# JiakangC/Neural-Network-Based-PDE-Solver

Measured on NVIDIA B200. Metric: collocation points/sec per train step (fwd+Δu+param-grad), higher is better.
Workload: dtype f32

## Files before the change

neural-network-based-pde-solver_b200/csrc/pde_tc.cu:

```cuda
#include <cuda_runtime.h>
#include <stdint.h>
#include <stdio.h>
#include <stdlib.h>
#include <string.h>
#include <atomic>
#include <type_traits>

#include "pde_launch.h"
#include "pde_tc.h"
#include "pde_tc_core.cuh"

namespace pde {
namespace tc {

constexpr int TP = 64;
constexpr int HP = 64;
constexpr int NEPI = 8;
constexpr int NE = 4;
constexpr int NTHREADS = (NEPI + 4) * 32;
constexpr int MAXC = 6;
constexpr int COL_R0 = 0;
constexpr int COL_G = 384;
constexpr int COL_SMALL = 448;

struct TcArgs {
  int n_h, act, H;
  const float* params;
  const unsigned char* wimg;
  const float* X;
  long long n;
  int num_tiles;
  int prog, n_q, want_grad;
  EnvDev<float> env;
  float alpha, beta_const, energy_const, inv_n;
  const float* f;
  const float* beta;
  const float* energy;
  const float* seed;
// ... 221 lines not shown
    }
  }
  if constexpr (ORDER == 2) {
    n0b += LB * lapb;
    nj[1 + ND] = B * lapb;
  }
  nj[0] = n0b;
}

template <int D, int C>
struct SmemMap {
  static constexpr int LIMIT = 232448;
  static constexpr int set_bytes = 2 * C * TILE_BYTES;
  static constexpr int par_floats = D * 64 + 4 * 64 + 64 + 4;
  static constexpr int red_floats = (2 * 64 * C > 256) ? 2 * 64 * C : 256;
  static constexpr int rest = 4096 + 1024 * (D > 0 ? D : 1) + par_floats * 4 + 64 * D * 4 + 64 * C * 4 + red_floats * 4 + 128;
  static constexpr int shadow_if = 2 * C * 2048;
  static constexpr bool fits3 = 2 * set_bytes + 3 * 2 * TILE_BYTES + shadow_if + rest <= LIMIT;
  static constexpr bool fits2 = 2 * set_bytes + 2 * 2 * TILE_BYTES + shadow_if + rest <= LIMIT;
  static constexpr bool shadow = (C <= 5) && (fits3 || fits2);
  static constexpr int w_slots = (C <= 5) ? ((shadow && !fits3) ? 2 : 3) : 1;
  static constexpr int off_T1 = 0;
  static constexpr int off_T2 = off_T1 + set_bytes;
  static constexpr int off_W = off_T2 + set_bytes;
  static constexpr int w_bytes = w_slots * 2 * TILE_BYTES;
  static constexpr int off_Z0 = off_W + w_bytes;
  static constexpr int off_XT = off_Z0 + (shadow ? shadow_if : 0);
  static constexpr int off_E = off_XT + 4096;
  static constexpr int off_par = off_E + 1024 * (D > 0 ? D : 1);
  static constexpr int off_X = off_par + par_floats * 4;
  static constexpr int off_nb = off_X + 64 * D * 4;
  static constexpr int off_red = off_nb + 64 * C * 4;
  static constexpr int off_bar = off_red + red_floats * 4;
  static constexpr int total = off_bar + 128;
  static_assert(total <= LIMIT, "shared-memory plan does not fit");
};

__device__ __forceinline__ void sts32(uint32_t addr, uint32_t v) { asm volatile("st.shared.b32 [%0], %1;" ::"r"(addr), "r"(v) : "memory"); }
__device__ __forceinline__ void stsm_x4(uint32_t addr, uint32_t r0, uint32_t r1, uint32_t r2, uint32_t r3) {
  asm volatile("stmatrix.sync.aligned.m8n8.x4.shared.b16 [%0], {%1,%2,%3,%4};" ::"r"(addr), "r"(r0), "r"(r1), "r"(r2), "r"(r3) : "memory");
}
__device__ __forceinline__ uint64_t l2_policy_evict_last() {
  uint64_t p;
  asm volatile("createpolicy.fractional.L2::evict_last.b64 %0, 1.0;" : "=l"(p));
  return p;
}
__device__ __forceinline__ uint64_t l2_policy_evict_first() {
  uint64_t p;
  asm volatile("createpolicy.fractional.L2::evict_first.b64 %0, 1.0;" : "=l"(p));
  return p;
}
__device__ __forceinline__ void stash_store(float4* p, float4 v, uint64_t pol) {
  asm volatile("st.global.cg.L2::cache_hint.v4.f32 [%0], {%1,%2,%3,%4}, %5;" ::"l"(p), "f"(v.x), "f"(v.y), "f"(v.z), "f"(v.w), "l"(pol) : "memory");
// ... 89 lines not shown
  uint64_t* bar_chunk = reinterpret_cast<uint64_t*>(sm + SM::off_bar);
  uint64_t* bar_d = bar_chunk + 4;
  uint64_t* bar_w = bar_chunk + 5;
  uint64_t* bar_own = bar_chunk + 6;
  uint64_t* bar_wt = bar_chunk + 7;
  uint32_t* tmem_slot = reinterpret_cast<uint32_t*>(bar_chunk + 8);
  int* sTileEnd = reinterpret_cast<int*>(bar_chunk + 14);
  float* sMx = reinterpret_cast<float*>(bar_chunk + 10);

  const int tid = threadIdx.x, warp = tid >> 5, lane = tid & 31;
  const int n_h = a.n_h;
  constexpr int act = ACT;
  const bool do_bwd = a.want_grad != 0;
  const uint32_t sbase = smem_u32(sm);
  const uint32_t sT1 = sbase + SM::off_T1, sT2 = sbase + SM::off_T2, sWT = sbase + SM::off_W;
  const uint32_t sXT = sbase + SM::off_XT, sET = sbase + SM::off_E, sZ0 = sbase + SM::off_Z0;

  auto w_addr = [&](int l) { return sWT + (WS == 3 ? l - 1 : (WS == 2 ? (l == 2 ? 0 : 1) : 0)) * 2 * TILE_BYTES; };
  for (int i = tid; i < D * 64 + n_h * 64; i += NTHREADS) sPar[i] = a.params[i];
  for (int i = tid; i < 64 + 1; i += NTHREADS) sWL[i] = a.params[D * 64 + n_h * 64 + i];
  if (tid == 0 && a.mode == 0) {
    sWL[65] = a.energy ? a.energy[0] : a.energy_const;
    sWL[66] = (a.seed ? a.seed[0] : 1.f) * a.inv_n;
    sWL[67] = (a.seed && a.prog == PDE_PROG_RAYLEIGH ? a.seed[1] : 1.f) * a.inv_n;
  }
  for (int i = tid; i < (1024 * (D > 0 ? D : 1)) / 4; i += NTHREADS) {
    const int n = i / 256, w = i % 256;
    reinterpret_cast<uint32_t*>(sm + SM::off_E)[i] = ((w >> 5) == n) ? ONE_X2 : 0u;
  }
  for (int i = tid; i < 1024; i += NTHREADS) {
    const int t = (i / 256) & 1, w = i % 256;
    reinterpret_cast<uint32_t*>(sm + SM::off_XT)[i] = (t == 0 && (w >> 5) == D) ? ONE_X2 : 0u;
  }
  {
    const uint4* src = reinterpret_cast<const uint4*>(a.wimg);
    uint4* dst = reinterpret_cast<uint4*>(sm + SM::off_W);
    for (int l = 1; l <= (n_h - 1 < WS ? n_h - 1 : WS); ++l) {
      dst = reinterpret_cast<uint4*>(sm + SM::off_W + (w_addr(l) - sWT));
      for (int i = tid; i < 2 * TILE_BYTES / 16; i += NTHREADS) dst[i] = src[(l - 1) * (2 * TILE_BYTES / 16) + i];
    }
  }
  if (tid == 0) {
    for (int j = 0; j < 4; ++j) mbar_init(&bar_chunk[j], NEPI);
    mbar_init(bar_d, 1);
    mbar_init(bar_w, 1);
    mbar_init(bar_own, 1);
    mbar_init(bar_wt, 1);
// ... 28 lines not shown
    }
  };
#else
  auto TS = [](int) {};
  auto TSW = [](int) {};
#endif
  auto d_addr = [&](int r, int c) { return taddr_of(tmem, 16 * (c & 1), COL_R0 + 192 * r + 64 * (c >> 1)); };

  if (warp >= NEPI) {
    asm volatile("setmaxnreg.dec.sync.aligned.u32 88;");
    if (warp == NEPI) {
      constexpr uint32_t ID_FWD = make_idesc(64, 64, 0, 0);
      constexpr uint32_t ID_FWD2 = make_idesc(128, 64, 0, 0), ID_DG2 = make_idesc(128, 64, 0, 1);
      constexpr uint32_t ID_DG = make_idesc(64, 64, 0, 1);
      constexpr uint32_t ID_WG = make_idesc(64, 64, 1, 1);
      constexpr uint32_t ID_SM = make_idesc(64, 8, 1, 0);
      constexpr uint32_t TD = TILE_BYTES >> 4;
      const uint32_t tm = __shfl_sync(0xffffffffu, tmem, 0);
      const uint32_t kT1K = (sT1 >> 4) | DESC_K_LBO, kT1M = (sT1 >> 4) | DESC_MN_LBO;
      const uint32_t kT2K = (sT2 >> 4) | DESC_K_LBO, kT2M = (sT2 >> 4) | DESC_MN_LBO;
      const uint32_t kXT0 = (sXT >> 4) | DESC_K_LBO, kETK = (sET >> 4) | DESC_K_LBO;
      uint32_t ph_chunk = 0, ph_own = 0, ph_wt = 0;
      int reg = 0;
      int cur_w = 1;
      const uint32_t kZ0 = (sZ0 >> 4) | ((128u >> 4) << 16);
      constexpr uint32_t DESC_HI_Z0 = (256u >> 4) | (1u << 14);
      bool w_loading = false;
      auto start_w_load = [&](int l) {
        if (elect_one()) {
          asm volatile("mbarrier.arrive.expect_tx.shared::cta.b64 _, [%0], %1;" ::"r"(smem_u32(bar_wt)), "r"(2 * TILE_BYTES) : "memory");
          asm volatile("cp.async.bulk.shared::cluster.global.mbarrier::complete_tx::bytes [%0], [%1], %2, [%3];" ::"r"(w_addr(l)),
                       "l"(a.wimg + (size_t)(l - 1) * 2 * TILE_BYTES), "r"(2 * TILE_BYTES), "r"(smem_u32(bar_wt))
                       : "memory");
        }
        __syncwarp();
        cur_w = l;
// ... 3 lines not shown
        if (WRES) return;
        if (WS == 2 && l == 2) return;
        if (cur_w != l) {
          if (elect_one()) mma_commit(bar_own);
          __syncwarp();
          mbar_wait(bar_own, ph_own);
          ph_own ^= 1;
          start_w_load(l);
        }
        if (w_loading) {
          mbar_wait(bar_wt, ph_wt);
          ph_wt ^= 1;
          w_loading = false;
        }
      };
      for (int tile = tile_begin; tile < tile_end; ++tile) {
        for (int l = 1; l < n_h; ++l) {
          uint32_t kT1K_ = kT1K, kT1M_ = kT1M, kT2K_ = kT2K, kT2M_ = kT2M, kXT0_ = kXT0, kETK_ = kETK, kZ0_ = kZ0;
          if constexpr (C <= 4) asm volatile("" : "+r"(kT1K_), "+r"(kT1M_), "+r"(kT2K_), "+r"(kT2M_), "+r"(kXT0_), "+r"(kETK_), "+r"(kZ0_));
          const uint32_t kW = (w_addr(l) >> 4) | DESC_K_LBO;
          const uint32_t dbase = tm + COL_R0 + 192 * reg;
          need_w(l);
#pragma unroll
          for (int j = 0; j < 4; ++j) {
            mbar_wait(&bar_chunk[j], ph_chunk);
            tc_fence_after();
            TS(100 + 10 * l + j);
            if (WS == 2 && j == 0 && l == 2 && n_h - 1 == 3) start_w_load(3);
            if (elect_one()) {
#pragma unroll
              for (int c = 0; c < C; ++c) {
                if (ch_paired(c, C) && (c & 1)) continue;
                const uint32_t d = dbase + 64 * (c >> 1);
                const uint32_t ah = kT1K_ + (ch_base(c, C) >> 4) + 2 * j, al = ah + (ch_lo(c, C) >> 4);
                const uint32_t id = ch_paired(c, C) ? ID_FWD2 : ID_FWD;
                mma_k(d, ah, DESC_HI, kW + 2 * j, DESC_HI, id, j > 0 ? 1u : 0u);
                mma_k(d, al, DESC_HI, kW + 2 * j, DESC_HI, id, 1u);
                mma_k(d, ah, DESC_HI, kW + TD + 2 * j, DESC_HI, id, 1u);
              }
            }
            __syncwarp();
          }
          if (elect_one()) mma_commit(bar_d);
          __syncwarp();
          ph_chunk ^= 1;
          reg ^= 1;
        }
        if (!do_bwd) continue;
        for (int l = n_h - 1; l >= 1; --l) {
          uint32_t kT1K_ = kT1K, kT1M_ = kT1M, kT2K_ = kT2K, kT2M_ = kT2M, kXT0_ = kXT0, kETK_ = kETK, kZ0_ = kZ0;
          if constexpr (C <= 4) asm volatile("" : "+r"(kT1K_), "+r"(kT1M_), "+r"(kT2K_), "+r"(kT2M_), "+r"(kXT0_), "+r"(kETK_), "+r"(kZ0_));
          const uint32_t kW = (w_addr(l) >> 4) | DESC_MN_LBO;
          const uint32_t dbase = tm + COL_R0 + 192 * reg;
          need_w(l);
#pragma unroll
          for (int j = 0; j < 4; ++j) {
            mbar_wait(&bar_chunk[j], ph_chunk);
            tc_fence_after();
            TS(200 + 10 * l + j);
            if (WS == 2 && j == 0 && l == 2 && n_h - 1 == 3) start_w_load(1);
            if (SHADOW && j == 0 && l < n_h - 1) {
              if (elect_one()) {
#pragma unroll
                for (int c = 0; c < C; ++c) {
                  if (ch_paired(c, C) && (c & 1)) continue;
                  const uint32_t d = dbase + 64 * (c >> 1);
// ... 34 lines not shown
#pragma unroll
              for (int ks = 0; ks < 4; ++ks) {
                const uint32_t zh = kT2M_ + ((ch_base(c, C) + ks * ch_kstep_mn(c, C)) >> 4), zl = zh + (ch_lo(c, C) >> 4);
                const uint32_t ah = kT1M_ + ((ch_base(c, C) + ks * ch_kstep_mn(c, C)) >> 4), al = ah + (ch_lo(c, C) >> 4);
                mma_k(d, zl, ch_hi_mn(c, C), ah, ch_hi_mn(c, C), ID_WG, (c == 0 && ks == 0) ? 0u : 1u);
                mma_k(d, zh, ch_hi_mn(c, C), al, ch_hi_mn(c, C), ID_WG, 1u);
              }
            }
#pragma unroll
            for (int c = 0; c < C; ++c) {
#pragma unroll
              for (int ks = 0; ks < 4; ++ks)
                mma_k(d, kT2M_ + ((ch_base(c, C) + ks * ch_kstep_mn(c, C)) >> 4), ch_hi_mn(c, C),
                      kT1M_ + ((ch_base(c, C) + ks * ch_kstep_mn(c, C)) >> 4), ch_hi_mn(c, C), ID_WG, 1u);
            }
            const uint32_t db = tm + (16u << 16) + COL_SMALL + 8 * l;
#pragma unroll
            for (int ks = 0; ks < 4; ++ks)
              mma_k(db, kT2M_ + ((ch_lo(0, C) + ks * ch_kstep_mn(0, C)) >> 4), ch_hi_mn(0, C), kETK_ + 2 * ks, DESC_HI, ID_SM, ks == 0 ? 0u : 1u);
#pragma unroll
            for (int ks = 0; ks < 4; ++ks) mma_k(db, kT2M_ + ((ks * ch_kstep_mn(0, C)) >> 4), ch_hi_mn(0, C), kETK_ + 2 * ks, DESC_HI, ID_SM, 1u);
            mma_commit(bar_w);
          }
          __syncwarp();
          if (refill_next) {
            mbar_wait(bar_own, ph_own);
            ph_own ^= 1;
            start_w_load(l - 1);
          }
        }
        {
          uint32_t kT1K_ = kT1K, kT1M_ = kT1M, kT2K_ = kT2K, kT2M_ = kT2M, kXT0_ = kXT0, kETK_ = kETK, kZ0_ = kZ0;
          if constexpr (C <= 4) asm volatile("" : "+r"(kT1K_), "+r"(kT1M_), "+r"(kT2K_), "+r"(kT2M_), "+r"(kXT0_), "+r"(kETK_), "+r"(kZ0_));
#pragma unroll
          for (int j = 0; j < 4; ++j) mbar_wait(&bar_chunk[j], ph_chunk);
          tc_fence_after();
          ph_chunk ^= 1;
          if (elect_one()) {
            const uint32_t d = tm + (16u << 16) + COL_SMALL;
            const uint32_t kXTK = kXT0_ + ((tile & 1) << 7);
#pragma unroll
            for (int ks = 0; ks < 4; ++ks) {
              mma_k(d, kT2M_ + ((ch_lo(0, C) + ks * ch_kstep_mn(0, C)) >> 4), ch_hi_mn(0, C), kXTK + 2 * ks, DESC_HI, ID_SM, ks == 0 ? 0u : 1u);
              mma_k(d, kT2M_ + ((ks * ch_kstep_mn(0, C)) >> 4), ch_hi_mn(0, C), kXTK + 64 + 2 * ks, DESC_HI, ID_SM, 1u);
            }
#pragma unroll
            for (int i = 0; i < ND; ++i) {
#pragma unroll
              for (int ks = 0; ks < 4; ++ks)
                mma_k(d, kT2M_ + ((ch_base(1 + i, C) + ch_lo(1 + i, C) + ks * ch_kstep_mn(1 + i, C)) >> 4), ch_hi_mn(1 + i, C),
                      kETK_ + 64 * (dir0 + i) + 2 * ks, DESC_HI, ID_SM, 1u);
            }
#pragma unroll
            for (int ks = 0; ks < 4; ++ks) mma_k(d, kT2M_ + ((ks * ch_kstep_mn(0, C)) >> 4), ch_hi_mn(0, C), kXTK + 2 * ks, DESC_HI, ID_SM, 1u);
#pragma unroll
            for (int i = 0; i < ND; ++i) {
#pragma unroll
              for (int ks = 0; ks < 4; ++ks)
                mma_k(d, kT2M_ + ((ch_base(1 + i, C) + ks * ch_kstep_mn(1 + i, C)) >> 4), ch_hi_mn(1 + i, C),
                      kETK_ + 64 * (dir0 + i) + 2 * ks, DESC_HI, ID_SM, 1u);
            }
            mma_commit(bar_w);
          }
          __syncwarp();
        }
      }
    }
  } else {
    asm volatile("setmaxnreg.inc.sync.aligned.u32 208;");
    const int q = warp & 3, h = (warp >> 2) & 1;
    int rows[2];
    rows[0] = 16 * q + (lane >> 2);
    rows[1] = rows[0] + 8;
    const int cq = 2 * (lane & 3);
    const int sm_row = 16 * q + 8 * ((lane >> 3) & 1) + (lane & 7);
    const int sm_tile = lane >> 4;
    const uint32_t sm_base = (uint32_t)(sm_tile * TILE_BYTES) + ((sm_row >> 3) << 10) + ((sm_row & 7) << 7);
    const int sm_r7 = sm_row & 7;
    float* part = a.partial + (long long)blockIdx.x * a.PP;
// ... 4 lines not shown
    };
    auto pick_ch = [&](const float (&t)[C][4], const int c, float (&v)[NE]) {
      if (ch_paired(c, C)) {
        const int p = c & ~1, k = 2 * (c & 1);
        v[0] = t[p][k]; v[1] = t[p][k + 1]; v[2] = t[p + 1][k]; v[3] = t[p + 1][k + 1];
      } else {
        pick(t[c], v);
      }
    };
    uint64_t pol_stash = 0, pol_stream = 0;
    pol_stash = l2_policy_evict_last();
    pol_stream = l2_policy_evict_first();
    uint32_t ph_d = 0, ph_w = 0;
    int reg = 0;
    bool w_pending = false;

    double qs[4] = {0.0, 0.0, 0.0, 0.0};
    double gE = 0.0;
    constexpr bool PARK_Q = (C == 6);
    const uint32_t qpark = taddr_of(tmem, 32 * q + 16, COL_SMALL + 32);
    auto q_load = [&](double (&t)[4], double& g) {
      uint32_t w0[4], w1[4];
      tmem_ld_16x256b_u32(qpark, w0);
      tmem_ld_16x256b_u32(qpark + 8, w1);
      tmem_ld_wait();
      t[0] = __hiloint2double((int)w0[1], (int)w0[0]);
      t[1] = __hiloint2double((int)w0[3], (int)w0[2]);
      t[2] = t[3] = 0.0;
      g = __hiloint2double((int)w1[1], (int)w1[0]);
    };
    auto q_store = [&](const double (&t)[4], const double g) {
      const uint32_t w0[4] = {(uint32_t)__double2loint(t[0]), (uint32_t)__double2hiint(t[0]), (uint32_t)__double2loint(t[1]), (uint32_t)__double2hiint(t[1])};
      const uint32_t w1[4] = {(uint32_t)__double2loint(g), (uint32_t)__double2hiint(g), 0u, 0u};
      tmem_st_16x256b_u32(qpark, w0);
      tmem_st_16x256b_u32(qpark + 8, w1);
// ... 52 lines not shown
      put_chunk(set, j, pk);
    };
    int chunk_pending = 0;
    auto chunk_done = [&](int j) {
      fence_proxy_async();
      tc_fence_before();
      __syncwarp();
      if (lane == 0) {
        for (int jj = chunk_pending; jj <= j; ++jj) mbar_arrive(&bar_chunk[jj]);
      }
      chunk_pending = (j + 1) & 3;
    };
    auto stash_at = [&](int l, int j, int v) { return stash + ((l * 4 + j) * NEPI * NV + v) * 32; };

    float accW[3][4][NE];
    float accB[3][2];
    float acc0[NE];
#pragma unroll
    for (int i = 0; i < 3; ++i) {
#pragma unroll
      for (int b = 0; b < 4; ++b)
#pragma unroll
        for (int e = 0; e < NE; ++e) accW[i][b][e] = 0.f;
#pragma unroll
      for (int r = 0; r < 2; ++r) accB[i][r] = 0.f;
    }
#pragma unroll
    for (int e = 0; e < NE; ++e) acc0[e] = 0.f;
    auto flush_grads = [&]() {
#pragma unroll
      for (int sl = 0; sl < 3; ++sl) {
        if (sl + 1 < n_h) {
          const uint32_t d = taddr_of(tmem, 32 * q + 16 * (sl & 1), COL_G + 64 * (sl >> 1));
          float v[4][4], w[4];
#pragma unroll
          for (int b = 0; b < 4; ++b) tmem_ld_16x256b(d + 32 * h + 8 * b, v[b]);
          tmem_ld_16x256b(taddr_of(tmem, 32 * q + 16, COL_SMALL + 8 * (sl + 1)), w);
          tmem_ld_wait();
#pragma unroll
          for (int b = 0; b < 4; ++b) {
            float t[NE];
            pick(v[b], t);
#pragma unroll
            for (int e = 0; e < NE; ++e) accW[sl][b][e] += t[e];
          }
          float t[NE];
          pick(w, t);
#pragma unroll
          for (int r = 0; r < 2; ++r) accB[sl][r] += t[2 * r];
        }
      }
      {
        float w[4], t[NE];
        tmem_ld_16x256b(taddr_of(tmem, 32 * q + 16, COL_SMALL), w);
        tmem_ld_wait();
        pick(w, t);
#pragma unroll
        for (int e = 0; e < NE; ++e) acc0[e] += t[e];
      }
      tc_fence_before();
    };

    constexpr int XR = (TP * D + NEPI * 32 - 1) / (NEPI * 32);
    float xnext[XR];
    auto load_x = [&](int tile) {
#pragma unroll
      for (int k = 0; k < XR; ++k) {
        const int i = tid + k * NEPI * 32;
        const long long gp = (long long)tile * TP + i / D;
        xnext[k] = stream_load_if(a.X + gp * D + (i % D), pol_stream, i < TP * D && gp < a.n);
      }
    };
    if (tile_begin < tile_end) load_x(tile_begin);
    if (tid == 0) *sTileEnd = tile_end;
    named_sync(1, NEPI * 32);
    auto tile_end_s = [&]() {
      int v;
      asm volatile("ld.shared.s32 %0, [%1];" : "=r"(v) : "r"(smem_u32(sTileEnd)));
      return v;
    };
    for (int tile = tile_begin; tile < tile_end_s(); ++tile) {
      const long long base = (long long)tile * TP;
      TS(1);
      TSW(1);
      const uint32_t sXTb = sXT + ((tile & 1) << 11);
      named_sync(1, NEPI * 32);
      TS(3);
#pragma unroll
      for (int k = 0; k < XR; ++k)
        if (tid + k * NEPI * 32 < TP * D) sX[tid + k * NEPI * 32] = xnext[k];
      named_sync(1, NEPI * 32);
      TS(4);
      if (tile + 1 < tile_end_s()) load_x(tile + 1);
      const bool in_tile = tid < TP && base + tid < a.n;
      const float fv = stream_load_if(a.f ? a.f + base + tid : nullptr, pol_stream, in_tile && a.f != nullptr);
      const float bt_raw = stream_load_if(a.beta ? a.beta + base + tid : nullptr, pol_stream, in_tile && a.beta != nullptr);
      if (do_bwd) {
        for (int i = tid; i < D * 32; i += NEPI * 32) {
          const int j = i / 32, pp = 2 * (i % 32);
          uint32_t hi, lo;
          split2(sX[pp * D + j], sX[(pp + 1) * D + j], hi, lo);
          const uint32_t off = tile_off(j, pp >> 3) + ((pp & 7) << 1);
          sts32(sXTb + off, hi);
          sts32(sXTb + 1024 + off, lo);
        }
      }

      TS(5);
      float outacc[2][C];
#pragma unroll
      for (int r = 0; r < 2; ++r)
#pragma unroll
        for (int c = 0; c < C; ++c) outacc[r][c] = 0.f;

      auto fwd_layer = [&](auto l0_tag, auto last_tag, const int l) {
        constexpr bool L0 = decltype(l0_tag)::value, LAST = decltype(last_tag)::value;
        TS(10 + l);
        if constexpr (LAST) {
          if (w_pending) {
            mbar_wait(bar_w, ph_w);
            ph_w ^= 1;
            w_pending = false;
            tc_fence_after();
            flush_grads();
          }
        }
        if constexpr (!L0) {
          if constexpr (!SPLIT) {
            if (l == 1 && a.mode == 0 && tid < TP) envelope_point<D, ORDER>(a, sX + tid * D, sNb + tid * C);
          }
          mbar_wait(bar_d, ph_d);
          ph_d ^= 1;
          tc_fence_after();
        }
        TS(20 + l);
        float xr[2][D > 0 ? D : 1];
        if constexpr (L0) {
#pragma unroll
// ... 75 lines not shown
              av[0][e] = s0;
              float S = 0.f;
#pragma unroll
              for (int i = 0; i < ND; ++i) {
                av[1 + i][e] = s1 * z[1 + i][e];
                S = fmaf(z[1 + i][e], z[1 + i][e], S);
              }
              if constexpr (LAP) av[1 + ND][e] = fmaf(s1, z[1 + ND][e], s2 * S);
            }
          }
          if (!L0 && j < 3) {
#pragma unroll
            for (int c = 0; c < C; ++c) tmem_ld_16x256b(zsrc + ((16 * (c & 1)) << 16) + 64 * (c >> 1) + 16 * (j + 1), zr[c]);
          }
          if constexpr (!LAST) {
            if (l == 1) TS(320 + j);
            store_chunk(sT1, j, av);
            if (l == 1) TS(330 + j);
            chunk_done(j);
            if (l == 1) TS(340 + j);
          } else {
            const float w0v = sWL[u0], w1v = sWL[u0 + 1];
#pragma unroll
            for (int c = 0; c < C; ++c) {
#pragma unroll
              for (int r = 0; r < 2; ++r) outacc[r][c] = fmaf(w0v, av[c][2 * r], fmaf(w1v, av[c][2 * r + 1], outacc[r][c]));
            }
          }
        }
        if constexpr (!L0) reg ^= 1;
// ... 82 lines not shown
        TSW(4);
        mx = fmaxf(sMx[0], sMx[1]);
        const float sm = adj_scale * mx;
        if (mx > 1e-30f && mx < 3.0e38f && (adj_scale == 0.f || sm > 256.f || sm < 0.0625f)) {
          int ex = (int)((__float_as_uint(mx) >> 23) & 255u) - 126;
          ex = max(-60, min(60, ex));
          const float ns = __uint_as_float((uint32_t)(127 + 2 - ex) << 23);
          if (adj_scale != 0.f) {
            const float ratio = ns / adj_scale;
#pragma unroll
            for (int i = 0; i < 3; ++i) {
#pragma unroll
              for (int b = 0; b < 4; ++b)
#pragma unroll
                for (int e = 0; e < NE; ++e) accW[i][b][e] *= ratio;
#pragma unroll
              for (int r = 0; r < 2; ++r) accB[i][r] *= ratio;
            }
#pragma unroll
            for (int e = 0; e < NE; ++e) acc0[e] *= ratio;
#pragma unroll
            for (int j = 0; j < 4; ++j) { gwl[j][0] *= ratio; gwl[j][1] *= ratio; }
            gbl *= ratio;
          }
          adj_scale = ns;
        }
        cur_scale = (adj_scale != 0.f) ? adj_scale : 1.f;
        if (tid < TP) gbl += nj[0] * cur_scale;
      }

      auto bwd_layer = [&](auto top_tag, auto lk_tag, const int l) {
        constexpr bool TOP = decltype(top_tag)::value;
        constexpr int LK = decltype(lk_tag)::value;
        float4 cur[NV], prv[NV];
        auto load_cur = [&](int j) {
// ... 25 lines not shown
        TS(40 + l);
        float nbr[2][C];
        if constexpr (TOP) {
#pragma unroll
          for (int r = 0; r < 2; ++r)
#pragma unroll
            for (int c = 0; c < C; ++c) nbr[r][c] = sNb[rows[r] * C + c] * cur_scale;
        }
        float abr[C][4];
        float ab[C][NE];
        const uint32_t absrc = d_addr(reg, 0) + ((32 * q) << 16) + 8 * h;
        if constexpr (!TOP) {
#pragma unroll
          for (int c = 0; c < C; ++c) tmem_ld_16x256b(absrc + ((16 * (c & 1)) << 16) + 64 * (c >> 1), abr[c]);
        }
        auto refill = [&](const int u0, float (&ap)[C][NE]) {
          float pv0[NE], pv1[NE];
          to_arr(prv[0], pv0);
          to_arr(prv[1], pv1);
          float zp[C][NE];
          if constexpr (LK >= 2) {
#pragma unroll
            for (int c = 1; c < C; ++c) to_arr(prv[1 + c], zp[c]);
          } else {
#pragma unroll
            for (int e = 0; e < NE; ++e) {
              const int u = u0 + (e & 1);
#pragma unroll
              for (int i = 0; i < ND; ++i) zp[1 + i][e] = sW0t[(dir0 + i) * 64 + u];
              if constexpr (LAP) zp[1 + ND][e] = 0.f;
// ... 144 lines not shown
  #pragma unroll
                  for (int i = 0; i < ND; ++i) g = fmaf(nbr[r][1 + i], s1 * zj[1 + i][e], g);
                  if constexpr (LAP) g = fmaf(nbr[r][1 + ND], fmaf(s1, zj[1 + ND][e], s2 * S), g);
                  gwl[j][e & 1] += g;
                }
              }
                      }
}
          if (j < 3) {
            if constexpr (!TOP) {
#pragma unroll
              for (int c = 0; c < C; ++c) tmem_ld_16x256b(absrc + ((16 * (c & 1)) << 16) + 64 * (c >> 1) + 16 * (j + 1), abr[c]);
            }
            load_cur(j + 1);
          }
          pack_chunk(zb, zk);
          }
          float ap[C][NE];
          if (REFILL) {
            refill(u0, ap);
            if (j < 3) load_prv(j + 1);
          }
          constexpr bool SHP0 = SH && LK == 0;
          if (j == (SH ? (SHP0 ? 2 : 1) : 0) && w_pending) {
            TS(50 + l);
            mbar_wait(bar_w, ph_w);
            ph_w ^= 1;
            w_pending = false;
            TS(60 + l);
          }
          if constexpr (SHP0) {
            if (j <= 2) {
              if (j == 0) {
                put_shadow(zk);
              } else if (j == 1) {
#pragma unroll
                for (int c = 0; c < C; ++c) tmem_st_16x256b_u32(park + 8 * c, zk[c]);
                tmem_st_wait();
              } else {
                put_chunk(sT2, 2, zk);
                uint32_t pk[C][NE];
#pragma unroll
                for (int c = 0; c < C; ++c) tmem_ld_16x256b_u32(park + 8 * c, pk[c]);
                tmem_ld_wait();
                put_chunk(sT2, 1, pk);
                copy_shadow();
                chunk_done(2);
              }
              continue;
            }
          }
          if (SH && j == 0) {
            put_shadow(zk);
            if constexpr (REFILL) {
              uint32_t pk[C][NE];
              pack_chunk(ap, pk);
#pragma unroll
              for (int c = 0; c < C; ++c) tmem_st_16x256b_u32(park + 8 * c, pk[c]);
              tmem_st_wait();
            }
          } else {
            put_chunk(sT2, j, zk);
            if constexpr (REFILL) store_chunk(sT1, j, ap);
            if constexpr (SH) if (j == 1) {
              if constexpr (REFILL) {
                uint32_t pk[C][NE];
#pragma unroll
                for (int c = 0; c < C; ++c) tmem_ld_16x256b_u32(park + 8 * c, pk[c]);
                tmem_ld_wait();
                put_chunk(sT1, 0, pk);
              }
              copy_shadow();
            }
          }
          chunk_done(j);
        }
        if constexpr (!TOP) reg ^= 1;
        w_pending = true;
      };
      using I0 = std::integral_constant<int, 0>;
      using I1 = std::integral_constant<int, 1>;
      using I2 = std::integral_constant<int, 2>;
      if (n_h - 1 >= 2) bwd_layer(std::true_type{}, I2{}, n_h - 1);
      else bwd_layer(std::true_type{}, I1{}, n_h - 1);
      for (int l = n_h - 2; l >= 2; --l) bwd_layer(std::false_type{}, I2{}, l);
      if (n_h - 2 >= 1) bwd_layer(std::false_type{}, I1{}, 1);
      bwd_layer(std::false_type{}, I0{}, 0);
    }

    if (w_pending) {
      mbar_wait(bar_w, ph_w);
      ph_w ^= 1;
      tc_fence_after();
      flush_grads();
    }
    if (do_bwd) {
      const float inv = (adj_scale != 0.f) ? 1.f / adj_scale : 1.f;
#pragma unroll
      for (int sl = 0; sl < 3; ++sl) {
        if (sl + 1 < n_h) {
          float* gW = part + a.off_gW + (long long)sl * ((long long)HP * HP + HP);
#pragma unroll
          for (int b = 0; b < 4; ++b) {
            const int i0 = 32 * h + 8 * b + cq;
#pragma unroll
            for (int r = 0; r < 2; ++r)
              *reinterpret_cast<float2*>(gW + rows[r] * HP + i0) = make_float2(accW[sl][b][2 * r] * inv, accW[sl][b][2 * r + 1] * inv);
          }
          if (h == 0 && (lane & 3) == 0) {
#pragma unroll
            for (int r = 0; r < 2; ++r) gW[HP * HP + rows[r]] = accB[sl][r] * inv;
          }
        }
      }
      if (h == 0) {
#pragma unroll
        for (int e = 0; e < NE; ++e) {
          const int col = cq + (e & 1), o = rows[e >> 1];
          if (col < D) part[a.off_gW0 + o * D + col] = acc0[e] * inv;
          else if (col == D) part[a.off_gb0 + o] = acc0[e] * inv;
        }
      }
#pragma unroll
      for (int j = 0; j < 4; ++j)
#pragma unroll
        for (int k = 0; k < 2; ++k) {
          float v = gwl[j][k];
          v += __shfl_xor_sync(0xffffffffu, v, 4);
          v += __shfl_xor_sync(0xffffffffu, v, 8);
          v += __shfl_xor_sync(0xffffffffu, v, 16);
          gwl[j][k] = v;
        }
      named_sync(1, NEPI * 32);
      float* sRedW = sRed;
      if (lane < 4) {
#pragma unroll
        for (int j = 0; j < 4; ++j) {
          sRedW[q * 64 + 16 * j + 8 * h + cq] = gwl[j][0];
          sRedW[q * 64 + 16 * j + 8 * h + cq + 1] = gwl[j][1];
        }
      }
      named_sync(1, NEPI * 32);
      if (tid < 64) {
        const float v = (sRedW[tid] + sRedW[64 + tid]) + (sRedW[128 + tid] + sRedW[192 + tid]);
        part[a.off_gwL + tid] = v * inv;
      }
      named_sync(1, NEPI * 32);
      if (tid < 64) sRed[tid] = gbl;
      named_sync(1, NEPI * 32);
      if (tid == 0) {
        float v = 0.f;
        for (int i = 0; i < 64; ++i) v += sRed[i];
        part[a.off_gbL] = v * inv;
      }
    }
    named_sync(1, NEPI * 32);
    {
      double* dred = reinterpret_cast<double*>(sm + SM::off_T1);
      if (tid < TP) {
        if constexpr (PARK_Q) q_load(qs, gE);
// ... 495 lines not shown
```

neural-network-based-pde-solver_b200/csrc/pde_tc_core.cuh:

```cuda
#pragma once
#include <cuda_bf16.h>
#include <cuda_runtime.h>
#include <stdint.h>

namespace pde {
namespace tc {

constexpr int TILE_BYTES = 8192;

__device__ __forceinline__ uint32_t smem_u32(const void* p) {
  return static_cast<uint32_t>(__cvta_generic_to_shared(p));
}

__host__ __device__ __forceinline__ uint32_t tile_off(int r, int c) {
  return ((r >> 3) << 10) + ((r & 7) << 7) + (((c ^ (r & 7)) & 7) << 4);
}

__device__ __forceinline__ void mbar_init(uint64_t* bar, uint32_t count) {
  asm volatile("mbarrier.init.shared::cta.b64 [%0], %1;" ::"r"(smem_u32(bar)), "r"(count));
}
__device__ __forceinline__ void mbar_arrive(uint64_t* bar) {
  asm volatile("mbarrier.arrive.shared::cta.b64 _, [%0];" ::"r"(smem_u32(bar)) : "memory");
}
__device__ __forceinline__ uint32_t mbar_try_wait(uint64_t* bar, uint32_t parity) {
// ... 35 lines not shown
  d |= static_cast<uint64_t>(sbo_bytes >> 4) << 32;
  d |= static_cast<uint64_t>(1) << 46;
  d |= static_cast<uint64_t>(2) << 61;
  return d;
}
__device__ __forceinline__ uint64_t desc_kmajor(uint32_t tile_saddr, int ks) {
  return make_desc(tile_saddr + ks * 32, 16, 1024);
}
__device__ __forceinline__ uint64_t desc_mnmajor(uint32_t tile_saddr, int ks) {
  return make_desc(tile_saddr + ks * 2048, 8192, 1024);
}

#ifndef PDE_TC_FP16
#define PDE_TC_FP16 1
#endif
constexpr uint32_t ONE_X2 = PDE_TC_FP16 ? 0x3C003C00u : 0x3F803F80u;

__host__ __device__ constexpr uint32_t make_idesc(int M, int N, int a_mn_major, int b_mn_major) {
  return (1u << 4) | ((PDE_TC_FP16 ? 0u : 1u) << 7) | ((PDE_TC_FP16 ? 0u : 1u) << 10) | (static_cast<uint32_t>(a_mn_major) << 15) |
         (static_cast<uint32_t>(b_mn_major) << 16) | (static_cast<uint32_t>(N >> 3) << 17) |
         (static_cast<uint32_t>(M >> 4) << 24);
}

__device__ __forceinline__ void mma_bf16(uint32_t d_tmem, uint64_t a_desc, uint64_t b_desc, uint32_t idesc, uint32_t accumulate) {
  asm volatile(
      "{\n\t"
      ".reg .pred p;\n\t"
      "setp.ne.b32 p, %4, 0;\n\t"
      "tcgen05.mma.cta_group::1.kind::f16 [%0], %1, %2, %3, p;\n\t"
      "}" ::"r"(d_tmem),
      "l"(a_desc), "l"(b_desc), "r"(idesc), "r"(accumulate)
// ... 76 lines not shown
```

Baseline: 416.2 million.

## Compute first-layer and bias gradients on CUDA cores instead of small MMAs

Removes the tensor-core MMAs that reduced bias and first-layer weight gradients against identity/ones matrices (the XT and E smem tiles and their per-tile split/store). The epilogue warps now compute those sums in FP32 with warp shuffles, accumulate them in registers (parked in TMEM when C==6), and reduce across warps through shared memory. The first layer's backward no longer packs chunks or triggers an MMA wait, and the grad-flush wait moves earlier in the forward pass. This frees MMA issue slots, smem and the extra sync in exchange for more shuffle and ALU work on the epilogue warps.

```diff
diff --git a/neural-network-based-pde-solver_b200/csrc/pde_tc.cu b/neural-network-based-pde-solver_b200/csrc/pde_tc.cu
--- a/neural-network-based-pde-solver_b200/csrc/pde_tc.cu
+++ b/neural-network-based-pde-solver_b200/csrc/pde_tc.cu
@@ -21,7 +21,7 @@
 constexpr int MAXC = 6;
 constexpr int COL_R0 = 0;
 constexpr int COL_G = 384;
-constexpr int COL_SMALL = 448;
+constexpr int COL_PARK = 448;
 
 struct TcArgs {
   int n_h, act, H;
@@ -273,7 +273,8 @@
   static constexpr int set_bytes = 2 * C * TILE_BYTES;
   static constexpr int par_floats = D * 64 + 4 * 64 + 64 + 4;
   static constexpr int red_floats = (2 * 64 * C > 256) ? 2 * 64 * C : 256;
-  static constexpr int rest = 4096 + 1024 * (D > 0 ? D : 1) + par_floats * 4 + 64 * D * 4 + 64 * C * 4 + red_floats * 4 + 128;
+  static constexpr int reserve = 4096 + 1024 * (D > 0 ? D : 1);
+  static constexpr int rest = reserve + par_floats * 4 + 64 * D * 4 + 64 * C * 4 + red_floats * 4 + 128;
   static constexpr int shadow_if = 2 * C * 2048;
   static constexpr bool fits3 = 2 * set_bytes + 3 * 2 * TILE_BYTES + shadow_if + rest <= LIMIT;
   static constexpr bool fits2 = 2 * set_bytes + 2 * 2 * TILE_BYTES + shadow_if + rest <= LIMIT;
@@ -284,9 +285,7 @@
   static constexpr int off_W = off_T2 + set_bytes;
   static constexpr int w_bytes = w_slots * 2 * TILE_BYTES;
   static constexpr int off_Z0 = off_W + w_bytes;
-  static constexpr int off_XT = off_Z0 + (shadow ? shadow_if : 0);
-  static constexpr int off_E = off_XT + 4096;
-  static constexpr int off_par = off_E + 1024 * (D > 0 ? D : 1);
+  static constexpr int off_par = off_Z0 + (shadow ? shadow_if : 0);
   static constexpr int off_X = off_par + par_floats * 4;
   static constexpr int off_nb = off_X + 64 * D * 4;
   static constexpr int off_red = off_nb + 64 * C * 4;
@@ -295,7 +294,6 @@
   static_assert(total <= LIMIT, "shared-memory plan does not fit");
 };
 
-__device__ __forceinline__ void sts32(uint32_t addr, uint32_t v) { asm volatile("st.shared.b32 [%0], %1;" ::"r"(addr), "r"(v) : "memory"); }
 __device__ __forceinline__ void stsm_x4(uint32_t addr, uint32_t r0, uint32_t r1, uint32_t r2, uint32_t r3) {
   asm volatile("stmatrix.sync.aligned.m8n8.x4.shared.b16 [%0], {%1,%2,%3,%4};" ::"r"(addr), "r"(r0), "r"(r1), "r"(r2), "r"(r3) : "memory");
 }
@@ -415,7 +413,7 @@
   const bool do_bwd = a.want_grad != 0;
   const uint32_t sbase = smem_u32(sm);
   const uint32_t sT1 = sbase + SM::off_T1, sT2 = sbase + SM::off_T2, sWT = sbase + SM::off_W;
-  const uint32_t sXT = sbase + SM::off_XT, sET = sbase + SM::off_E, sZ0 = sbase + SM::off_Z0;
+  const uint32_t sZ0 = sbase + SM::off_Z0;
 
   auto w_addr = [&](int l) { return sWT + (WS == 3 ? l - 1 : (WS == 2 ? (l == 2 ? 0 : 1) : 0)) * 2 * TILE_BYTES; };
   for (int i = tid; i < D * 64 + n_h * 64; i += NTHREADS) sPar[i] = a.params[i];
@@ -424,14 +422,6 @@
     sWL[65] = a.energy ? a.energy[0] : a.energy_const;
     sWL[66] = (a.seed ? a.seed[0] : 1.f) * a.inv_n;
     sWL[67] = (a.seed && a.prog == PDE_PROG_RAYLEIGH ? a.seed[1] : 1.f) * a.inv_n;
-  }
-  for (int i = tid; i < (1024 * (D > 0 ? D : 1)) / 4; i += NTHREADS) {
-    const int n = i / 256, w = i % 256;
-    reinterpret_cast<uint32_t*>(sm + SM::off_E)[i] = ((w >> 5) == n) ? ONE_X2 : 0u;
-  }
-  for (int i = tid; i < 1024; i += NTHREADS) {
-    const int t = (i / 256) & 1, w = i % 256;
-    reinterpret_cast<uint32_t*>(sm + SM::off_XT)[i] = (t == 0 && (w >> 5) == D) ? ONE_X2 : 0u;
   }
   {
     const uint4* src = reinterpret_cast<const uint4*>(a.wimg);
@@ -490,12 +480,10 @@
       constexpr uint32_t ID_FWD2 = make_idesc(128, 64, 0, 0), ID_DG2 = make_idesc(128, 64, 0, 1);
       constexpr uint32_t ID_DG = make_idesc(64, 64, 0, 1);
       constexpr uint32_t ID_WG = make_idesc(64, 64, 1, 1);
-      constexpr uint32_t ID_SM = make_idesc(64, 8, 1, 0);
       constexpr uint32_t TD = TILE_BYTES >> 4;
       const uint32_t tm = __shfl_sync(0xffffffffu, tmem, 0);
       const uint32_t kT1K = (sT1 >> 4) | DESC_K_LBO, kT1M = (sT1 >> 4) | DESC_MN_LBO;
       const uint32_t kT2K = (sT2 >> 4) | DESC_K_LBO, kT2M = (sT2 >> 4) | DESC_MN_LBO;
-      const uint32_t kXT0 = (sXT >> 4) | DESC_K_LBO, kETK = (sET >> 4) | DESC_K_LBO;
       uint32_t ph_chunk = 0, ph_own = 0, ph_wt = 0;
       int reg = 0;
       int cur_w = 1;
@@ -529,10 +517,10 @@
           w_loading = false;
         }
       };
-      for (int tile = tile_begin; tile < tile_end; ++tile) {
+      for (int tiles_left = tile_end - tile_begin; tiles_left > 0; --tiles_left) {
         for (int l = 1; l < n_h; ++l) {
-          uint32_t kT1K_ = kT1K, kT1M_ = kT1M, kT2K_ = kT2K, kT2M_ = kT2M, kXT0_ = kXT0, kETK_ = kETK, kZ0_ = kZ0;
-          if constexpr (C <= 4) asm volatile("" : "+r"(kT1K_), "+r"(kT1M_), "+r"(kT2K_), "+r"(kT2M_), "+r"(kXT0_), "+r"(kETK_), "+r"(kZ0_));
+          uint32_t kT1K_ = kT1K, kT1M_ = kT1M, kT2K_ = kT2K, kT2M_ = kT2M, kZ0_ = kZ0;
+          if constexpr (C <= 4) asm volatile("" : "+r"(kT1K_), "+r"(kT1M_), "+r"(kT2K_), "+r"(kT2M_), "+r"(kZ0_));
           const uint32_t kW = (w_addr(l) >> 4) | DESC_K_LBO;
           const uint32_t dbase = tm + COL_R0 + 192 * reg;
           need_w(l);
@@ -563,8 +551,8 @@
         }
         if (!do_bwd) continue;
         for (int l = n_h - 1; l >= 1; --l) {
-          uint32_t kT1K_ = kT1K, kT1M_ = kT1M, kT2K_ = kT2K, kT2M_ = kT2M, kXT0_ = kXT0, kETK_ = kETK, kZ0_ = kZ0;
-          if constexpr (C <= 4) asm volatile("" : "+r"(kT1K_), "+r"(kT1M_), "+r"(kT2K_), "+r"(kT2M_), "+r"(kXT0_), "+r"(kETK_), "+r"(kZ0_));
+          uint32_t kT1K_ = kT1K, kT1M_ = kT1M, kT2K_ = kT2K, kT2M_ = kT2M, kZ0_ = kZ0;
+          if constexpr (C <= 5) asm volatile("" : "+r"(kT1K_), "+r"(kT1M_), "+r"(kT2K_), "+r"(kT2M_), "+r"(kZ0_));
           const uint32_t kW = (w_addr(l) >> 4) | DESC_MN_LBO;
           const uint32_t dbase = tm + COL_R0 + 192 * reg;
           need_w(l);
@@ -629,12 +617,6 @@
                 mma_k(d, kT2M_ + ((ch_base(c, C) + ks * ch_kstep_mn(c, C)) >> 4), ch_hi_mn(c, C),
                       kT1M_ + ((ch_base(c, C) + ks * ch_kstep_mn(c, C)) >> 4), ch_hi_mn(c, C), ID_WG, 1u);
             }
-            const uint32_t db = tm + (16u << 16) + COL_SMALL + 8 * l;
-#pragma unroll
-            for (int ks = 0; ks < 4; ++ks)
-              mma_k(db, kT2M_ + ((ch_lo(0, C) + ks * ch_kstep_mn(0, C)) >> 4), ch_hi_mn(0, C), kETK_ + 2 * ks, DESC_HI, ID_SM, ks == 0 ? 0u : 1u);
-#pragma unroll
-            for (int ks = 0; ks < 4; ++ks) mma_k(db, kT2M_ + ((ks * ch_kstep_mn(0, C)) >> 4), ch_hi_mn(0, C), kETK_ + 2 * ks, DESC_HI, ID_SM, 1u);
             mma_commit(bar_w);
           }
           __syncwarp();
@@ -643,41 +625,6 @@
             ph_own ^= 1;
             start_w_load(l - 1);
           }
-        }
-        {
-          uint32_t kT1K_ = kT1K, kT1M_ = kT1M, kT2K_ = kT2K, kT2M_ = kT2M, kXT0_ = kXT0, kETK_ = kETK, kZ0_ = kZ0;
-          if constexpr (C <= 4) asm volatile("" : "+r"(kT1K_), "+r"(kT1M_), "+r"(kT2K_), "+r"(kT2M_), "+r"(kXT0_), "+r"(kETK_), "+r"(kZ0_));
-#pragma unroll
-          for (int j = 0; j < 4; ++j) mbar_wait(&bar_chunk[j], ph_chunk);
-          tc_fence_after();
-          ph_chunk ^= 1;
-          if (elect_one()) {
-            const uint32_t d = tm + (16u << 16) + COL_SMALL;
-            const uint32_t kXTK = kXT0_ + ((tile & 1) << 7);
-#pragma unroll
-            for (int ks = 0; ks < 4; ++ks) {
-              mma_k(d, kT2M_ + ((ch_lo(0, C) + ks * ch_kstep_mn(0, C)) >> 4), ch_hi_mn(0, C), kXTK + 2 * ks, DESC_HI, ID_SM, ks == 0 ? 0u : 1u);
-              mma_k(d, kT2M_ + ((ks * ch_kstep_mn(0, C)) >> 4), ch_hi_mn(0, C), kXTK + 64 + 2 * ks, DESC_HI, ID_SM, 1u);
-            }
-#pragma unroll
-            for (int i = 0; i < ND; ++i) {
-#pragma unroll
-              for (int ks = 0; ks < 4; ++ks)
-                mma_k(d, kT2M_ + ((ch_base(1 + i, C) + ch_lo(1 + i, C) + ks * ch_kstep_mn(1 + i, C)) >> 4), ch_hi_mn(1 + i, C),
-                      kETK_ + 64 * (dir0 + i) + 2 * ks, DESC_HI, ID_SM, 1u);
-            }
-#pragma unroll
-            for (int ks = 0; ks < 4; ++ks) mma_k(d, kT2M_ + ((ks * ch_kstep_mn(0, C)) >> 4), ch_hi_mn(0, C), kXTK + 2 * ks, DESC_HI, ID_SM, 1u);
-#pragma unroll
-            for (int i = 0; i < ND; ++i) {
-#pragma unroll
-              for (int ks = 0; ks < 4; ++ks)
-                mma_k(d, kT2M_ + ((ch_base(1 + i, C) + ks * ch_kstep_mn(1 + i, C)) >> 4), ch_hi_mn(1 + i, C),
-                      kETK_ + 64 * (dir0 + i) + 2 * ks, DESC_HI, ID_SM, 1u);
-            }
-            mma_commit(bar_w);
-          }
-          __syncwarp();
         }
       }
     }
@@ -712,11 +659,12 @@
     uint32_t ph_d = 0, ph_w = 0;
     int reg = 0;
     bool w_pending = false;
+    bool flush_due = false;
 
     double qs[4] = {0.0, 0.0, 0.0, 0.0};
     double gE = 0.0;
     constexpr bool PARK_Q = (C == 6);
-    const uint32_t qpark = taddr_of(tmem, 32 * q + 16, COL_SMALL + 32);
+    const uint32_t qpark = taddr_of(tmem, 32 * q + 16, COL_PARK + 32);
     auto q_load = [&](double (&t)[4], double& g) {
       uint32_t w0[4], w1[4];
       tmem_ld_16x256b_u32(qpark, w0);
@@ -799,28 +747,47 @@
     auto stash_at = [&](int l, int j, int v) { return stash + ((l * 4 + j) * NEPI * NV + v) * 32; };
 
     float accW[3][4][NE];
-    float accB[3][2];
-    float acc0[NE];
+    float accB[3];
+    constexpr int N0 = (2 * (D + 1) + 7) / 8 * 8, K0 = N0 / 8;
+    float acc0[4][K0];
+    const uint32_t park0 = taddr_of(tmem, 32 * q + 16, COL_PARK + 16 * h);
+    static_assert(!PARK_Q || K0 == 2, "acc0 parks as two 16x256b fragments");
+    auto acc0_load = [&]() {
+      float w0[4], w1[4];
+      tmem_ld_16x256b(park0, w0);
+      tmem_ld_16x256b(park0 + 8, w1);
+#pragma unroll
+      for (int f = 0; f < 4; ++f) { acc0[f / 2][f % 2] = w0[f]; acc0[2 + f / 2][f % 2] = w1[f]; }
+    };
+    auto acc0_store = [&]() {
+      uint32_t w0[4], w1[4];
+#pragma unroll
+      for (int f = 0; f < 4; ++f) { w0[f] = __float_as_uint(acc0[f / 2][f % 2]); w1[f] = __float_as_uint(acc0[2 + f / 2][f % 2]); }
+      tmem_st_16x256b_u32(park0, w0);
+      tmem_st_16x256b_u32(park0 + 8, w1);
+      tmem_st_wait();
+    };
 #pragma unroll
     for (int i = 0; i < 3; ++i) {
 #pragma unroll
       for (int b = 0; b < 4; ++b)
 #pragma unroll
         for (int e = 0; e < NE; ++e) accW[i][b][e] = 0.f;
-#pragma unroll
-      for (int r = 0; r < 2; ++r) accB[i][r] = 0.f;
+      accB[i] = 0.f;
     }
 #pragma unroll
-    for (int e = 0; e < NE; ++e) acc0[e] = 0.f;
+    for (int j = 0; j < 4; ++j)
+#pragma unroll
+      for (int k = 0; k < K0; ++k) acc0[j][k] = 0.f;
+    if constexpr (PARK_Q) acc0_store();
     auto flush_grads = [&]() {
 #pragma unroll
       for (int sl = 0; sl < 3; ++sl) {
         if (sl + 1 < n_h) {
           const uint32_t d = taddr_of(tmem, 32 * q + 16 * (sl & 1), COL_G + 64 * (sl >> 1));
-          float v[4][4], w[4];
+          float v[4][4];
 #pragma unroll
           for (int b = 0; b < 4; ++b) tmem_ld_16x256b(d + 32 * h + 8 * b, v[b]);
-          tmem_ld_16x256b(taddr_of(tmem, 32 * q + 16, COL_SMALL + 8 * (sl + 1)), w);
           tmem_ld_wait();
 #pragma unroll
           for (int b = 0; b < 4; ++b) {
@@ -829,21 +796,61 @@
 #pragma unroll
             for (int e = 0; e < NE; ++e) accW[sl][b][e] += t[e];
           }
-          float t[NE];
-          pick(w, t);
-#pragma unroll
-          for (int r = 0; r < 2; ++r) accB[sl][r] += t[2 * r];
-        }
-      }
-      {
-        float w[4], t[NE];
-        tmem_ld_16x256b(taddr_of(tmem, 32 * q + 16, COL_SMALL), w);
-        tmem_ld_wait();
-        pick(w, t);
-#pragma unroll
-        for (int e = 0; e < NE; ++e) acc0[e] += t[e];
+        }
       }
       tc_fence_before();
+    };
+
+    auto first_layer_sums = [&](const float (&zb)[C][NE], const int j) {
+      float x[2][D > 0 ? D : 1];
+#pragma unroll
+      for (int r = 0; r < 2; ++r)
+#pragma unroll
+        for (int jd = 0; jd < D; ++jd) x[r][jd] = sX[rows[r] * D + jd];
+      float v[N0];
+#pragma unroll
+      for (int e1 = 0; e1 < 2; ++e1) {
+        const float za = zb[0][e1], zc = zb[0][2 + e1];
+        v[e1 * (D + 1) + D] = za + zc;
+#pragma unroll
+        for (int jd = 0; jd < D; ++jd) {
+          float t = fmaf(zc, x[1][jd], za * x[0][jd]);
+#pragma unroll
+          for (int i = 0; i < ND; ++i)
+            if (jd == dir0 + i) t += zb[1 + i][e1] + zb[1 + i][2 + e1];
+          v[e1 * (D + 1) + jd] = t;
+        }
+      }
+#pragma unroll
+      for (int t = 2 * (D + 1); t < N0; ++t) v[t] = 0.f;
+#pragma unroll
+      for (int m = 16, n = N0 / 2; m >= 4; m >>= 1, n >>= 1) {
+        const bool up = (lane & m) != 0;
+#pragma unroll
+        for (int i = 0; i < n; ++i) {
+          const float keep = up ? v[i + n] : v[i], send = up ? v[i] : v[i + n];
+          v[i] = keep + __shfl_xor_sync(0xffffffffu, send, m);
+        }
+      }
+#pragma unroll
+      for (int jj = 0; jj < 4; ++jj)
+        if (jj == j) {
+#pragma unroll
+          for (int k = 0; k < K0; ++k) acc0[jj][k] += v[k];
+        }
+    };
+
+    auto bias_sums = [&](const float (&zb)[C][NE], const int j, const int sl) {
+      const float b0 = zb[0][0] + zb[0][2], b1 = zb[0][1] + zb[0][3];
+      const bool up = (lane & 16) != 0;
+      float v = (up ? b1 : b0) + __shfl_xor_sync(0xffffffffu, up ? b0 : b1, 16);
+      v += __shfl_xor_sync(0xffffffffu, v, 8);
+      v += __shfl_xor_sync(0xffffffffu, v, 4);
+      if (((lane >> 2) & 3) == j) {
+#pragma unroll
+        for (int i = 0; i < 3; ++i)
+          if (i == sl) accB[i] += v;
+      }
     };
 
     constexpr int XR = (TP * D + NEPI * 32 - 1) / (NEPI * 32);
@@ -868,7 +875,6 @@
       const long long base = (long long)tile * TP;
       TS(1);
       TSW(1);
-      const uint32_t sXTb = sXT + ((tile & 1) << 11);
       named_sync(1, NEPI * 32);
       TS(3);
 #pragma unroll
@@ -880,16 +886,6 @@
       const bool in_tile = tid < TP && base + tid < a.n;
       const float fv = stream_load_if(a.f ? a.f + base + tid : nullptr, pol_stream, in_tile && a.f != nullptr);
       const float bt_raw = stream_load_if(a.beta ? a.beta + base + tid : nullptr, pol_stream, in_tile && a.beta != nullptr);
-      if (do_bwd) {
-        for (int i = tid; i < D * 32; i += NEPI * 32) {
-          const int j = i / 32, pp = 2 * (i % 32);
-          uint32_t hi, lo;
-          split2(sX[pp * D + j], sX[(pp + 1) * D + j], hi, lo);
-          const uint32_t off = tile_off(j, pp >> 3) + ((pp & 7) << 1);
-          sts32(sXTb + off, hi);
-          sts32(sXTb + 1024 + off, lo);
-        }
-      }
 
       TS(5);
       float outacc[2][C];
@@ -902,11 +898,8 @@
         constexpr bool L0 = decltype(l0_tag)::value, LAST = decltype(last_tag)::value;
         TS(10 + l);
         if constexpr (LAST) {
-          if (w_pending) {
-            mbar_wait(bar_w, ph_w);
-            ph_w ^= 1;
-            w_pending = false;
-            tc_fence_after();
+          if (flush_due) {
+            flush_due = false;
             flush_grads();
           }
         }
@@ -1012,6 +1005,15 @@
             for (int c = 0; c < C; ++c) tmem_ld_16x256b(zsrc + ((16 * (c & 1)) << 16) + 64 * (c >> 1) + 16 * (j + 1), zr[c]);
           }
           if constexpr (!LAST) {
+            if (L0 && j == 0 && w_pending) {
+              TS(7);
+              mbar_wait(bar_w, ph_w);
+              ph_w ^= 1;
+              w_pending = false;
+              flush_due = true;
+              tc_fence_after();
+              TS(8);
+            }
             if (l == 1) TS(320 + j);
             store_chunk(sT1, j, av);
             if (l == 1) TS(330 + j);
@@ -1124,11 +1126,17 @@
               for (int b = 0; b < 4; ++b)
 #pragma unroll
                 for (int e = 0; e < NE; ++e) accW[i][b][e] *= ratio;
-#pragma unroll
-              for (int r = 0; r < 2; ++r) accB[i][r] *= ratio;
-            }
-#pragma unroll
-            for (int e = 0; e < NE; ++e) acc0[e] *= ratio;
+              accB[i] *= ratio;
+            }
+            if constexpr (PARK_Q) {
+              acc0_load();
+              tmem_ld_wait();
+            }
+#pragma unroll
+            for (int j = 0; j < 4; ++j)
+#pragma unroll
+              for (int k = 0; k < K0; ++k) acc0[j][k] *= ratio;
+            if constexpr (PARK_Q) acc0_store();
 #pragma unroll
             for (int j = 0; j < 4; ++j) { gwl[j][0] *= ratio; gwl[j][1] *= ratio; }
             gbl *= ratio;
@@ -1184,6 +1192,7 @@
 #pragma unroll
           for (int c = 0; c < C; ++c) tmem_ld_16x256b(absrc + ((16 * (c & 1)) << 16) + 64 * (c >> 1), abr[c]);
         }
+        if constexpr (PARK_Q && LK == 0) acc0_load();
         auto refill = [&](const int u0, float (&ap)[C][NE]) {
           float pv0[NE], pv1[NE];
           to_arr(prv[0], pv0);
@@ -1358,41 +1367,25 @@
             }
             load_cur(j + 1);
           }
-          pack_chunk(zb, zk);
-          }
+          if constexpr (LK == 0) {
+            first_layer_sums(zb, j);
+          } else {
+            bias_sums(zb, j, LK == 1 ? 0 : l - 1);
+            pack_chunk(zb, zk);
+          }
+          }
+          if constexpr (LK == 0) continue;
           float ap[C][NE];
           if (REFILL) {
             refill(u0, ap);
             if (j < 3) load_prv(j + 1);
           }
-          constexpr bool SHP0 = SH && LK == 0;
-          if (j == (SH ? (SHP0 ? 2 : 1) : 0) && w_pending) {
+          if (j == (SH ? 1 : 0) && w_pending) {
             TS(50 + l);
             mbar_wait(bar_w, ph_w);
             ph_w ^= 1;
             w_pending = false;
             TS(60 + l);
-          }
-          if constexpr (SHP0) {
-            if (j <= 2) {
-              if (j == 0) {
-                put_shadow(zk);
-              } else if (j == 1) {
-#pragma unroll
-                for (int c = 0; c < C; ++c) tmem_st_16x256b_u32(park + 8 * c, zk[c]);
-                tmem_st_wait();
-              } else {
-                put_chunk(sT2, 2, zk);
-                uint32_t pk[C][NE];
-#pragma unroll
-                for (int c = 0; c < C; ++c) tmem_ld_16x256b_u32(park + 8 * c, pk[c]);
-                tmem_ld_wait();
-                put_chunk(sT2, 1, pk);
-                copy_shadow();
-                chunk_done(2);
-              }
-              continue;
-            }
           }
           if (SH && j == 0) {
             put_shadow(zk);
@@ -1420,7 +1413,8 @@
           chunk_done(j);
         }
         if constexpr (!TOP) reg ^= 1;
-        w_pending = true;
+        if constexpr (PARK_Q && LK == 0) acc0_store();
+        if constexpr (LK >= 1) w_pending = true;
       };
       using I0 = std::integral_constant<int, 0>;
       using I1 = std::integral_constant<int, 1>;
@@ -1451,20 +1445,23 @@
             for (int r = 0; r < 2; ++r)
               *reinterpret_cast<float2*>(gW + rows[r] * HP + i0) = make_float2(accW[sl][b][2 * r] * inv, accW[sl][b][2 * r + 1] * inv);
           }
-          if (h == 0 && (lane & 3) == 0) {
-#pragma unroll
-            for (int r = 0; r < 2; ++r) gW[HP * HP + rows[r]] = accB[sl][r] * inv;
-          }
-        }
-      }
-      if (h == 0) {
-#pragma unroll
-        for (int e = 0; e < NE; ++e) {
-          const int col = cq + (e & 1), o = rows[e >> 1];
-          if (col < D) part[a.off_gW0 + o * D + col] = acc0[e] * inv;
-          else if (col == D) part[a.off_gb0 + o] = acc0[e] * inv;
-        }
-      }
+        }
+      }
+      float* sRed0 = reinterpret_cast<float*>(sm + SM::off_T2);
+      float* sRedB = sRed0 + 4 * 64 * (D + 1);
+      if constexpr (PARK_Q) {
+        acc0_load();
+        tmem_ld_wait();
+      }
+#pragma unroll
+      for (int j = 0; j < 4; ++j)
+#pragma unroll
+        for (int k = 0; k < K0; ++k) {
+          const int t = (lane >> 2) * K0 + k;
+          if (t < 2 * (D + 1)) sRed0[(q * 64 + 16 * j + 8 * h + cq + t / (D + 1)) * (D + 1) + t % (D + 1)] = acc0[j][k];
+        }
+#pragma unroll
+      for (int sl = 0; sl < 3; ++sl) sRedB[(q * 3 + sl) * 64 + 16 * (lane >> 2 & 3) + 8 * h + cq + (lane >> 4)] = accB[sl];
 #pragma unroll
       for (int j = 0; j < 4; ++j)
 #pragma unroll
@@ -1488,6 +1485,17 @@
       if (tid < 64) {
         const float v = (sRedW[tid] + sRedW[64 + tid]) + (sRedW[128 + tid] + sRedW[192 + tid]);
         part[a.off_gwL + tid] = v * inv;
+      }
+      for (int i = tid; i < 64 * (D + 1); i += NEPI * 32) {
+        constexpr int QS = 64 * (D + 1);
+        const float v = ((sRed0[i] + sRed0[QS + i]) + (sRed0[2 * QS + i] + sRed0[3 * QS + i])) * inv;
+        const int o = i / (D + 1), col = i % (D + 1);
+        if (col < D) part[a.off_gW0 + o * D + col] = v;
+        else part[a.off_gb0 + o] = v;
+      }
+      for (int i = tid; i < (n_h - 1) * 64; i += NEPI * 32) {
+        const float v = ((sRedB[i] + sRedB[192 + i]) + (sRedB[384 + i] + sRedB[576 + i])) * inv;
+        part[a.off_gW + (long long)(i / 64) * ((long long)HP * HP + HP) + HP * HP + i % 64] = v;
       }
       named_sync(1, NEPI * 32);
       if (tid < 64) sRed[tid] = gbl;
diff --git a/neural-network-based-pde-solver_b200/csrc/pde_tc_core.cuh b/neural-network-based-pde-solver_b200/csrc/pde_tc_core.cuh
--- a/neural-network-based-pde-solver_b200/csrc/pde_tc_core.cuh
+++ b/neural-network-based-pde-solver_b200/csrc/pde_tc_core.cuh
@@ -73,7 +73,6 @@
 #ifndef PDE_TC_FP16
 #define PDE_TC_FP16 1
 #endif
-constexpr uint32_t ONE_X2 = PDE_TC_FP16 ? 0x3C003C00u : 0x3F803F80u;
 
 __host__ __device__ constexpr uint32_t make_idesc(int M, int N, int a_mn_major, int b_mn_major) {
   return (1u << 4) | ((PDE_TC_FP16 ? 0u : 1u) << 7) | ((PDE_TC_FP16 ? 0u : 1u) << 10) | (static_cast<uint32_t>(a_mn_major) << 15) |
```

Result: faster. 425.3 million, median of 6 (+2.2%).
